# Repeerc/flash-attention-v2-RDNA3-minimal

Hardware: AMD Instinct MI355X
Metric: fwd attention TFLOPS (and % MFMA roofline) at B2 H16 N4096 D128 fp16 (higher is better)
Workload: dtype f16; 1 GPU; c2: B2 H16 N4096 D128 float16 causal=False per GPU, BHND, torch.rand U[0,1); global_batch=2, parallelism=batch-shard x1 (no data-path collective)

## Files before the change

### flash-attention-v2-rdna3-minimal_amd/build.py

```python
import argparse
import concurrent.futures
import fcntl
import hashlib
import os
import shutil
import subprocess
import sys
import tempfile

PKG_DIR = os.path.dirname(os.path.realpath(__file__))
REPO_ROOT = os.path.dirname(PKG_DIR)
CSRC = os.path.join(PKG_DIR, "csrc")
INCLUDE = os.path.join(REPO_ROOT, "include")
LIB_NAME = "libfa2_gfx950.so"
LIB_PATH = os.path.join(PKG_DIR, LIB_NAME)
STAMP_PATH = LIB_PATH + ".stamp"
LOCK_PATH = LIB_PATH + ".lock"

UNITS = [
    ("host", "host.cpp", []),
    ("fwd_hip_f16", "fwd_hip.cpp", ["-DFA2_TU_BF16=0"]),
    ("fwd_hip_bf16", "fwd_hip.cpp", ["-DFA2_TU_BF16=1"]),
    ("fwd_hip_trim_f16", "fwd_hip.cpp", ["-DFA2_TU_BF16=0", "-DFA2_TU_TRIM=1"]),
    ("fwd_hip_trim_bf16", "fwd_hip.cpp", ["-DFA2_TU_BF16=1", "-DFA2_TU_TRIM=1"]),
    ("fwd_asm", "fwd_asm.cpp", []),
    ("bwd_hip_f16", "bwd_hip.cpp", ["-DFA2_TU_BF16=0"]),
    ("bwd_hip_bf16", "bwd_hip.cpp", ["-DFA2_TU_BF16=1"]),
    ("bwd_hip_trim_f16", "bwd_hip.cpp", ["-DFA2_TU_BF16=0", "-DFA2_TU_TRIM=1"]),
    ("bwd_hip_trim_bf16", "bwd_hip.cpp", ["-DFA2_TU_BF16=1", "-DFA2_TU_TRIM=1"]),
    ("bwd_asm", "bwd_asm.cpp", []),
    ("bwd_bias_hip_f16", "bwd_bias_hip.cpp", ["-DFA2_TU_BF16=0"]),
    ("bwd_bias_hip_bf16", "bwd_bias_hip.cpp", ["-DFA2_TU_BF16=1"]),
    ("window_hip_f16", "window_hip.cpp", ["-DFA2_TU_BF16=0"]),
    ("window_hip_bf16", "window_hip.cpp", ["-DFA2_TU_BF16=1"]),
    ("varlen_hip_f16", "varlen_hip.cpp", ["-DFA2_TU_BF16=0"]),
    ("varlen_hip_bf16", "varlen_hip.cpp", ["-DFA2_TU_BF16=1"]),
    ("dropout_hip_f16", "dropout_hip.cpp", ["-DFA2_TU_BF16=0"]),
    ("dropout_hip_bf16", "dropout_hip.cpp", ["-DFA2_TU_BF16=1"]),
    ("varlen_dropout_hip_f16", "varlen_dropout_hip.cpp", ["-DFA2_TU_BF16=0"]),
    ("varlen_dropout_hip_bf16", "varlen_dropout_hip.cpp", ["-DFA2_TU_BF16=1"]),
    ("scoremod_hip_f16", "scoremod_hip.cpp", ["-DFA2_TU_BF16=0"]),
    ("scoremod_hip_bf16", "scoremod_hip.cpp", ["-DFA2_TU_BF16=1"]),
    ("varlen_scoremod_hip_f16", "varlen_scoremod_hip.cpp", ["-DFA2_TU_BF16=0"]),
    ("varlen_scoremod_hip_bf16", "varlen_scoremod_hip.cpp", ["-DFA2_TU_BF16=1"]),
]
FRONTEND_SRC = "frontend.cpp"
FRONTEND_PATH = os.path.join(PKG_DIR, "rocwmma_fattn", "_fa2_frontend.so")
GENERATORS = [os.path.join("gen", "fwd_d128_gen.py"), os.path.join("gen", "fwd_m16_gen.py"), os.path.join("gen", "fwd_m16_d256_gen.py"), os.path.join("gen", "bwd_d128_gen.py"),
              os.path.join("gen", "bwd_dq_m16_gen.py"), os.path.join("gen", "bwd_dkv_m16_gen.py")]
HEADERS = ["fa2_launch.h", "fa2_window.h", "fa2_dropout.h", "fa2_scoremod.h", "fa2_fwd_kernel.hip.h", "fa2_fwd_short.hip.h", "fa2_fwd_d128.hip.h", "fa2_fwd_d256.hip.h", "fa2_bwd_kernel.hip.h", "fa2_bwd_short.hip.h", "fa2_bwd_d128.hip.h",
           os.path.join(INCLUDE, "fa2_gfx950.h"), os.path.join("gen", "isa.py"), os.path.join("gen", "sched.py")] + GENERATORS

HIPCC_FLAGS = [
    "-x", "hip",
    "--offload-arch=gfx950",
    "-O3",
    "-std=c++17",
    "-fPIC",
    "-fvisibility-inlines-hidden",
    "-fno-honor-nans",
    "--offload-compress",
]


def _hipcc():
    for cand in (os.environ.get("HIPCC"), shutil.which("hipcc"), "/opt/rocm/bin/hipcc"):
        if cand and os.path.exists(cand):
            return cand
    raise RuntimeError("hipcc not found (set HIPCC or install ROCm); the gfx950 library cannot be built")


def _existing(names):
    out = []
    for name in names:
        path = name if os.path.isabs(name) else os.path.join(CSRC, name)
        if os.path.exists(path):
            out.append(path)
    return out


def _source_digest():
    h = hashlib.sha256()
    h.update(" ".join(HIPCC_FLAGS).encode())
    for (obj, src, flags) in UNITS:
        h.update(("%s %s %s" % (obj, src, " ".join(flags))).encode())
    for path in _existing(sorted(set(u[1] for u in UNITS)) + HEADERS + [FRONTEND_SRC]):
        with open(path, "rb") as f:
            h.update(f.read())
    return h.hexdigest()


def _dir_digest(d):
    h = hashlib.sha256()
    for name in sorted(os.listdir(d)):
        if name.endswith(".inc"):
            h.update(name.encode())
            with open(os.path.join(d, name), "rb") as f:
                h.update(f.read())
    return h.hexdigest()


def generate(out_dir=None, opts=None, probe=False):
    out_dir = out_dir or CSRC
# ... 136 lines not shown
```

### flash-attention-v2-rdna3-minimal_amd/csrc/fa2_fwd_d128.hip.h

```cpp
#pragma once
#include "fa2_fwd_kernel.hip.h"

#ifndef FA2_D128_INC_DIR
#define FA2_D128_INC(name) #name
#else
#define FA2_D128_STR2(x) #x
#define FA2_D128_STR(x) FA2_D128_STR2(x)
#define FA2_D128_INC(name) FA2_D128_STR(FA2_D128_INC_DIR/name)
#endif

namespace fa2 {

template <int HD>
struct AsmGeo {
    static constexpr int ROWB = 2 * HD, TILEB = 64 * ROWB;
    static constexpr int EPI_ROWB = ROWB + 16;
    static constexpr int EPI_BASE = 4 * TILEB;
    static constexpr int FAIL_OFF = EPI_BASE + 4 * 64 * EPI_ROWB;
    static constexpr int LDS_BYTES = FAIL_OFF + 16;
    static constexpr int RPP = 1024 / ROWB;
};
constexpr int kD128LdsBytes = AsmGeo<128>::LDS_BYTES;

typedef uint32_t u32x4s __attribute__((ext_vector_type(4)));

struct D128Item {
    u32x4s qrs, krs, vrs;
    uint32_t qw;
    int lim[2];
    int ntw, ntiles;
    int b, h, qw0;
    int slot;
};

__device__ __forceinline__ int part_of_item(const FwdParams& p, int v, int& item, int& part) {
    item = v;
    part = -1;
    if (p.nsplit > 1 && v >= p.full_items) {
        const int j = v - p.full_items;
        part = j / p.split_items;
        item = p.full_items + j % p.split_items;
        return (j % p.split_items) * p.nsplit + part;
    }
    return -1;
}


__device__ __forceinline__ void causal_item(const FwdParams& p, int v, int& bh, int& qblk) {
    const int P = (p.nqblk + 1) >> 1;
    const int unit = v >> 1, part = v & 1;
    int head, i;
    if ((p.nbh & 7) == 0) { const int r = unit >> 3; head = (unit & 7) + 8 * (r / P); i = r % P; }
    else { head = unit / P; i = unit % P; }
    bh = head + p.bh0;
    qblk = part ? i : p.nqblk - 1 - i;
}
__device__ __forceinline__ bool causal_unit_has_second(const FwdParams& p, int v) {
    const int P = (p.nqblk + 1) >> 1, unit = v >> 1;
    const int i = ((p.nbh & 7) == 0 ? unit >> 3 : unit) % P;
    return 2 * i + 1 < p.nqblk;
}
template <int HD, bool BF16, bool CAUSAL, bool FOLD, bool M16 = false, bool LM = false>
__global__ __launch_bounds__(256, 1) void fwd_asm_kernel(const FwdParams p_in) {
    using AG = AsmGeo<HD>;
    using G_ = Geo<HD, 4>;
    extern __shared__ __attribute__((aligned(16))) char smem[];
    int vb = blockIdx.x;
    if constexpr (CAUSAL) {
        if (p_in.persist != 0) vb = 2 * blockIdx.x;
    }
#ifdef FA2_STAMP
    const uint64_t stamp0 = __builtin_amdgcn_s_memrealtime();
    const uint64_t cyc0 = __builtin_readcyclecounter();
#endif
    uint32_t staged = 0;
    if (threadIdx.x < 4) reinterpret_cast<volatile uint32_t*>(smem + AG::FAIL_OFF)[threadIdx.x] = 0;
    __syncthreads();
#pragma clang loop unroll(disable)
    do {
        int tid = threadIdx.x;
        asm volatile("" : "+v"(tid), "+s"(staged));
        const FwdParams& p = p_in;
        const int lane = tid & 63;
        const int wave = __builtin_amdgcn_readfirstlane(tid >> 6);
        const int l31 = lane & 31, hi = lane >> 5;
        int nitems = (CAUSAL && p.persist != 0) ? 2 * p.nbh * ((p.nqblk + 1) >> 1) : p.nbh * p.nqblk;
        if (!CAUSAL && p.item_cap > 0) nitems = p.item_cap;

        const uint32_t k_rowb = (uint32_t)p.ks[2] * 2u, v_rowb = (uint32_t)p.vs[2] * 2u, q_rowb = (uint32_t)p.qs[2] * 2u;
        const int drow = 16 * wave + lane / G_::G, dslot = lane % G_::G;
        const uint32_t kd0 = drow * k_rowb + ((dslot ^ ((drow / G_::RPB) & G_::KMASK)) << 4);
        const int qrow = lane / G_::G;
        const uint32_t qd0 = qrow * q_rowb + ((dslot ^ ((qrow / G_::RPB) & G_::KMASK)) << 4);
        const uint32_t q_t16 = 16u * q_rowb;
        const uint32_t vd0 = drow * v_rowb + (((((dslot >> 2) ^ ((drow / G_::RPB) & G_::VMASK)) << 2) |
                                               ((dslot & 3) ^ ((M16 && (FOLD || LM)) ? (((drow >> 2) & 1) << 1) : 0))) << 4);
        const int pp4 = lane & 15, g1 = (lane >> 4) & 1;
        const int n16 = lane & 15, g4 = lane >> 4;
        const int trow16 = 4 * g4 + (n16 >> 2);
        const uint32_t kr0 = M16 ? (uint32_t)(n16 * AG::ROWB + ((g4 ^ ((n16 / G_::RPB) & G_::KMASK)) << 4)) : (uint32_t)G_::k_off(l31, hi);
        const uint32_t vr0 = M16 ? (uint32_t)(trow16 * AG::ROWB + (((trow16 / G_::RPB) & G_::VMASK) << 6) + 8 * (n16 & 3) + ((FOLD || LM) ? 32 * (g4 & 1) : 0))
                                 : (uint32_t)G_::v_off(4 * hi + (pp4 >> 2), 32 * g1 + 8 * (pp4 & 3));
        const uint32_t epi = M16 ? AG::EPI_BASE + wave * 64 * AG::EPI_ROWB + n16 * AG::EPI_ROWB + g4 * 8
                                 : AG::EPI_BASE + wave * 64 * AG::EPI_ROWB + l31 * AG::EPI_ROWB + hi * 16;
        const uint32_t k_tile = kKvTile * k_rowb, v_tile = kKvTile * v_rowb, k_row4 = AG::RPP * k_rowb - 1024, v_row4 = AG::RPP * v_rowb - 1024;
        const uint32_t ldsw = wave * (AG::TILEB / 4);
        const float c = p.c;

        auto make_item = [&](int item) {
            D128Item it;
            int bh, qblk;
            int kv_first = 0, nkv = p.Nkv;
            it.slot = -1;
            if constexpr (CAUSAL) {
                if (p.persist != 0) causal_item(p, item, bh, qblk);
                else block_to_head_qblock<CAUSAL>(p, item, bh, qblk);
            } else {
                int whole, part;
                it.slot = part_of_item(p, item, whole, part);
                block_to_head_qblock<CAUSAL>(p, whole, bh, qblk);
                if (part >= 0) {
                    const int nt = (p.Nkv + kKvTile - 1) / kKvTile;
                    const int t0 = part * nt / p.nsplit, t1 = (part + 1) * nt / p.nsplit;
                    kv_first = t0 * kKvTile;
                    nkv = (t1 * kKvTile < p.Nkv ? t1 * kKvTile : p.Nkv) - kv_first;
                }
                kv_first = __builtin_amdgcn_readfirstlane(kv_first);
                nkv = __builtin_amdgcn_readfirstlane(nkv);
                bh = __builtin_amdgcn_readfirstlane(bh);
                qblk = __builtin_amdgcn_readfirstlane(qblk);
                it.slot = __builtin_amdgcn_readfirstlane(it.slot);
            }
            it.b = bh / p.H;
            it.h = bh % p.H;
            const int q0 = qblk * 256;
            it.qw0 = q0 + wave * 64;
            int ntiles = (nkv + kKvTile - 1) / kKvTile;
            if (CAUSAL) {
                const int qmax = (q0 + 256 < p.Nq ? q0 + 256 : p.Nq) - 1;
                const int nt_c = qmax / kKvTile + 1;
                ntiles = nt_c < ntiles ? nt_c : ntiles;
            }
            int ntw = ntiles;
            if (CAUSAL) {
                const int nt_w = (it.qw0 + 63) / kKvTile + 1;
                ntw = nt_w < ntiles ? nt_w : ntiles;
            }
            it.ntiles = ntiles;
            it.ntw = ntw;
            const uint64_t qa = (uint64_t)((const uint16_t*)p.q + it.b * p.qs[0] + it.h * p.qs[1]);
            it.qrs = (u32x4s){(uint32_t)qa, (uint32_t)(qa >> 32) & 0xffffu, (uint32_t)(p.Nq - 1) * q_rowb + 2u * (uint32_t)p.D, 0x00020000u};
            it.qw = __builtin_amdgcn_readfirstlane(it.qw0 < p.Nq ? (uint32_t)it.qw0 * q_rowb : 0u);
#pragma unroll
            for (int qb = 0; qb < 2; ++qb) {
                const int qrow = it.qw0 + 32 * qb + l31;
                const int lim_c = CAUSAL ? qrow : 0x3fffffff;
                it.lim[qb] = (lim_c < nkv - 1 ? lim_c : nkv - 1) - kKvTile * (ntw - 1) - 4 * hi;
            }
            if constexpr (M16) {
                it.lim[0] = (CAUSAL ? it.qw0 + n16 : 0x3fff0000) - kKvTile * (ntw - 1) - 4 * g4;
                it.lim[1] = nkv - 1 - kKvTile * (ntw - 1) - 4 * g4;
            }
            const uint64_t ka = (uint64_t)((const uint16_t*)p.k + it.b * p.ks[0] + (it.h / p.kv_group) * p.ks[1] + (int64_t)kv_first * p.ks[2]);
            const uint64_t va = (uint64_t)((const uint16_t*)p.v + it.b * p.vs[0] + (it.h / p.kv_group) * p.vs[1] + (int64_t)kv_first * p.vs[2]);
            it.krs = (u32x4s){(uint32_t)ka, (uint32_t)(ka >> 32) & 0xffffu, p.k_bytes - (uint32_t)kv_first * k_rowb, 0x00020000u};
            it.vrs = (u32x4s){(uint32_t)va, (uint32_t)(va >> 32) & 0xffffu, p.v_bytes - (uint32_t)kv_first * v_rowb, 0x00020000u};
            return it;
        };

        int nvb;
        if constexpr (CAUSAL) {
            if (p.persist == 0) nvb = nitems;
            else if (!(vb & 1) && causal_unit_has_second(p, vb)) nvb = vb + 1;
            else nvb = (vb | 1) - 1 + 2 * (int)gridDim.x;
        } else {
            nvb = vb + (int)gridDim.x;
        }
        const bool has_next = nvb < nitems;
        const D128Item cur = make_item(vb);
        const D128Item nxt = make_item(has_next ? nvb : vb);
        const uint32_t flags = __builtin_amdgcn_readfirstlane(staged | (has_next ? 2u : 0u) | (nxt.ntiles >= 2 ? 4u : 0u) | (cur.slot >= 0 ? 8u : 0u) |
                                                              ((M16 && p.D < HD) ? (uint32_t)(p.D >> 3) << 8 : 0u));
        const int slot_u = __builtin_amdgcn_readfirstlane(cur.slot >= 0 ? cur.slot : 0);
        const uint64_t ws_tile = (uint64_t)(p.ws + (int64_t)slot_u * kSplitRows * HD);
        float lse0, lse1;

#define FA2_D128_OPERANDS                                                                                              \
    : "=v"(lse0), "=v"(lse1)                                                                                           \
    : "v"(qd0), "s"(cur.qw), "s"(cur.qrs), "s"(cur.krs), "s"(cur.vrs), "v"(kd0), "v"(vd0), "v"(kr0), "v"(vr0), \
      "v"(cur.lim[0]), "v"(cur.lim[1]), "s"(c), "s"(cur.ntw), "s"(cur.ntiles), "s"(k_tile), "s"(v_tile), "s"(k_row4),    \
      "s"(v_row4), "s"(ldsw), "v"(epi), "s"(flags), "s"(nxt.qw), "s"(q_t16), "s"(nxt.qrs), "s"(nxt.krs),                \
      "s"(nxt.vrs), "s"(ws_tile)                                                                                        \
    :
        if constexpr (M16 && LM && !FOLD) {
            if constexpr (HD == 64 && BF16) {
                asm volatile(
#include FA2_D128_INC(fa2_fwd_m16_d64_bf16_lm.inc)
                    FA2_D128_OPERANDS
#include FA2_D128_INC(fa2_fwd_d128_clobbers.inc)
                );
            } else if constexpr (HD == 64) {
                asm volatile(
#include FA2_D128_INC(fa2_fwd_m16_d64_f16_lm.inc)
                    FA2_D128_OPERANDS
#include FA2_D128_INC(fa2_fwd_d128_clobbers.inc)
                );
            } else if constexpr (BF16) {
                asm volatile(
#include FA2_D128_INC(fa2_fwd_m16_bf16_lm.inc)
                    FA2_D128_OPERANDS
#include FA2_D128_INC(fa2_fwd_d128_clobbers.inc)
                );
            } else {
                asm volatile(
#include FA2_D128_INC(fa2_fwd_m16_f16_lm.inc)
                    FA2_D128_OPERANDS
#include FA2_D128_INC(fa2_fwd_d128_clobbers.inc)
                );
            }
        } else if constexpr (M16 && HD == 64 && BF16 && FOLD) {
            asm volatile(
#include FA2_D128_INC(fa2_fwd_m16_d64_bf16_fold.inc)
                FA2_D128_OPERANDS
#include FA2_D128_INC(fa2_fwd_d128_clobbers.inc)
            );
        } else if constexpr (M16 && HD == 64 && FOLD) {
            asm volatile(
#include FA2_D128_INC(fa2_fwd_m16_d64_f16_fold.inc)
                FA2_D128_OPERANDS
#include FA2_D128_INC(fa2_fwd_d128_clobbers.inc)
            );
        } else if constexpr (M16 && HD == 64 && BF16) {
            asm volatile(
#include FA2_D128_INC(fa2_fwd_m16_d64_bf16.inc)
                FA2_D128_OPERANDS
#include FA2_D128_INC(fa2_fwd_d128_clobbers.inc)
            );
        } else if constexpr (M16 && HD == 64) {
            asm volatile(
#include FA2_D128_INC(fa2_fwd_m16_d64_f16.inc)
                FA2_D128_OPERANDS
#include FA2_D128_INC(fa2_fwd_d128_clobbers.inc)
            );
// ... 33 lines not shown
                FA2_D128_OPERANDS
#include FA2_D128_INC(fa2_fwd_d128_clobbers.inc)
            );
        } else if constexpr (HD == 128 && BF16 && FOLD) {
            asm volatile(
#include FA2_D128_INC(fa2_fwd_d128_bf16_fold.inc)
                FA2_D128_OPERANDS
#include FA2_D128_INC(fa2_fwd_d128_clobbers.inc)
            );
        } else if constexpr (HD == 128 && BF16) {
            asm volatile(
#include FA2_D128_INC(fa2_fwd_d128_bf16.inc)
                FA2_D128_OPERANDS
#include FA2_D128_INC(fa2_fwd_d128_clobbers.inc)
            );
        } else if constexpr (HD == 128 && FOLD) {
            asm volatile(
#include FA2_D128_INC(fa2_fwd_d128_f16_fold.inc)
                FA2_D128_OPERANDS
#include FA2_D128_INC(fa2_fwd_d128_clobbers.inc)
            );
        } else if constexpr (HD == 128) {
            asm volatile(
#include FA2_D128_INC(fa2_fwd_d128_f16.inc)
                FA2_D128_OPERANDS
#include FA2_D128_INC(fa2_fwd_d128_clobbers.inc)
            );
        } else if constexpr (BF16 && FOLD) {
            asm volatile(
#include FA2_D128_INC(fa2_fwd_d64_bf16_fold.inc)
                FA2_D128_OPERANDS
#include FA2_D128_INC(fa2_fwd_d128_clobbers.inc)
            );
        } else if constexpr (BF16) {
            asm volatile(
#include FA2_D128_INC(fa2_fwd_d64_bf16.inc)
                FA2_D128_OPERANDS
#include FA2_D128_INC(fa2_fwd_d128_clobbers.inc)
            );
        } else if constexpr (FOLD) {
            asm volatile(
#include FA2_D128_INC(fa2_fwd_d64_f16_fold.inc)
                FA2_D128_OPERANDS
#include FA2_D128_INC(fa2_fwd_d128_clobbers.inc)
            );
        } else {
            asm volatile(
#include FA2_D128_INC(fa2_fwd_d64_f16.inc)
                FA2_D128_OPERANDS
#include FA2_D128_INC(fa2_fwd_d128_clobbers.inc)
            );
        }
#undef FA2_D128_OPERANDS

        int tid2 = threadIdx.x, item2 = vb;
        asm volatile("" : "+v"(tid2));
        {
            if constexpr (M16) __syncthreads();
            const u32x4 fw = *reinterpret_cast<const volatile u32x4*>(smem + AG::FAIL_OFF);
            const uint32_t fany = __builtin_amdgcn_readfirstlane(fw.x | fw.y | fw.z | fw.w);
            if (fany != 0) {
                __syncthreads();
                if (tid2 < 4) reinterpret_cast<volatile uint32_t*>(smem + AG::FAIL_OFF)[tid2] = 0;
                __syncthreads();
            }
            if ((fany & 1u) == 0 && fany != 0) staged = __builtin_amdgcn_readfirstlane(staged | 32u);
            if ((fany & 1u) != 0) {
                staged = __builtin_amdgcn_readfirstlane(16u | 32u);
                continue;
            }
        }
        {
            const FwdParams& p2 = p_in;
            const int lane2 = tid2 & 63, wave2 = __builtin_amdgcn_readfirstlane(tid2 >> 6);
            int bh, qblk, slot2 = -1;
            if constexpr (CAUSAL) {
                if (p2.persist != 0) causal_item(p2, item2, bh, qblk);
                else block_to_head_qblock<CAUSAL>(p2, item2, bh, qblk);
            } else {
                int whole, part;
                slot2 = part_of_item(p2, item2, whole, part);
                block_to_head_qblock<CAUSAL>(p2, whole, bh, qblk);
            }
            const int b = bh / p2.H, h = bh % p2.H;
            const int qw0 = qblk * 256 + wave2 * 64;
            {
                const bool is_part = slot2 >= 0;
                float* lp = is_part ? p2.ws + (int64_t)p2.split_items * p2.nsplit * kSplitRows * HD + (int64_t)slot2 * kSplitRows + wave2 * 64 - qw0
                                    : p2.lse + b * p2.ls[0] + h * p2.ls[1];
                if constexpr (M16) {
                    if (is_part || qw0 + lane2 < p2.Nq) lp[qw0 + lane2] = lse0;
                } else if ((lane2 >> 5) == 0) {
                    if (is_part || qw0 + (lane2 & 31) < p2.Nq) lp[qw0 + (lane2 & 31)] = lse0;
                    if (is_part || qw0 + 32 + (lane2 & 31) < p2.Nq) lp[qw0 + 32 + (lane2 & 31)] = lse1;
                }
            }
            const int nq_store = slot2 >= 0 ? 0 : p2.Nq;
            const char* img = smem + AG::EPI_BASE + wave2 * 64 * AG::EPI_ROWB;
            constexpr int LPR = HD / 8;
            const int rl = lane2 / LPR, cl = lane2 % LPR;
            uint16_t* obase = (uint16_t*)p2.o + b * p2.os[0] + h * p2.os[1];
#pragma unroll
            for (int i = 0; i < 64 / (64 / LPR); ++i) {
                const int r = i * (64 / LPR) + rl;
                const u32x4 w = *(const u32x4*)(img + r * AG::EPI_ROWB + cl * 16);
#ifdef FA2_O_NT
                if (qw0 + r < nq_store) __builtin_nontemporal_store(w, (u32x4*)(obase + (int64_t)(qw0 + r) * p2.os[2] + cl * 8));
#else
                if (qw0 + r < nq_store && cl * 8 < p2.D) *(u32x4*)(obase + (int64_t)(qw0 + r) * p2.os[2] + cl * 8) = w;
#endif
            }
            staged = __builtin_amdgcn_readfirstlane((has_next ? 1u : 0u) | ((staged & 32u) ? 48u : 0u));
            vb = nvb;
#ifdef FA2_STAMP
            if (!has_next && lane2 == 0) {
                __builtin_amdgcn_s_waitcnt(0);
                uint64_t* st = (uint64_t*)p2.lse + (blockIdx.x * 4 + wave2) * 4;
                st[0] = stamp0;
                st[1] = __builtin_amdgcn_s_memrealtime();
                st[2] = __builtin_readcyclecounter() - cyc0;
                st[3] = ((uint64_t)__builtin_amdgcn_s_getreg(6164) << 32) | __builtin_amdgcn_s_getreg(63492);
            }
#endif
            if (!has_next) break;
        }
    } while (true);
}

}
```

### flash-attention-v2-rdna3-minimal_amd/csrc/fa2_fwd_kernel.hip.h

```cpp
#pragma once
#include <hip/hip_runtime.h>
#include <stdint.h>
#include <type_traits>

#include "fa2_window.h"

#ifndef FA2_WIN
#define FA2_WIN 0
#endif
#ifndef FA2_VARLEN
#define FA2_VARLEN 0
#endif
#if FA2_VARLEN && !FA2_WIN
#error "FA2_VARLEN builds on the FA2_WIN blocks"
#endif
#if FA2_VARLEN
#define FA2_KP pk
#else
#define FA2_KP p
#endif
#ifndef FA2_DROP
#define FA2_DROP 0
#endif
#if FA2_DROP && !FA2_WIN
#error "FA2_DROP builds on the FA2_WIN blocks"
#endif
#if FA2_DROP
#include "fa2_dropout.h"
#endif
#ifndef FA2_SMOD
#define FA2_SMOD 0
#endif
#if FA2_SMOD && (!FA2_WIN || FA2_DROP)
#error "FA2_SMOD builds on the FA2_WIN blocks and does not combine with FA2_DROP"
#endif
#if FA2_SMOD
#include "fa2_scoremod.h"
#define FA2_SMOD_PARAM , const ScoreMod smod
#else
#define FA2_SMOD_PARAM
#endif

#ifndef FA2_DEFER_THR
#define FA2_DEFER_THR 8.0f
#endif
#ifndef FA2_LDS_DMA
#define FA2_LDS_DMA 1
#endif
#ifndef FA2_LDS_DMA_MIN_HD
#define FA2_LDS_DMA_MIN_HD 128
#endif
#ifndef FA2_EPI_LDS
#define FA2_EPI_LDS 1
#endif
#ifndef FA2_IGLP
#define FA2_IGLP 0
#endif
#ifndef FA2_TILE_IN_SOFFSET
#define FA2_TILE_IN_SOFFSET 1
#endif
#if FA2_TILE_IN_SOFFSET
#define FA2_TILE_OFF(voff, soff) (voff), (soff)
#else
#define FA2_TILE_OFF(voff, soff) (voff) + (soff), 0u
#endif

namespace fa2 {

typedef _Float16 f16x8 __attribute__((ext_vector_type(8)));
typedef __bf16 bf16x8 __attribute__((ext_vector_type(8)));
typedef _Float16 f16x2 __attribute__((ext_vector_type(2)));
typedef __bf16 bf16x2 __attribute__((ext_vector_type(2)));
typedef float f32x16 __attribute__((ext_vector_type(16)));
typedef float f32x2 __attribute__((ext_vector_type(2)));
typedef float f32x4 __attribute__((ext_vector_type(4)));
typedef uint32_t u32x4 __attribute__((ext_vector_type(4)));
typedef uint32_t u32x2 __attribute__((ext_vector_type(2)));
typedef short s16x4 __attribute__((ext_vector_type(4)));
typedef uint32_t u32x32 __attribute__((ext_vector_type(32)));

constexpr int kQBlock = 256;
constexpr int kKvTile = 64;
constexpr uint32_t kOobOffset = 0x80000000u;

struct FwdParams {
    const void* q;
    const void* k;
    const void* v;
    void* o;
    float* lse;
    int B, H, Nq, Nkv;
    int D;
    int64_t qs[3], ks[3], vs[3], os[3];
    int64_t ls[2];
    float c;
    int negate_q;
    int nqblk;
    uint32_t k_bytes, v_bytes;
    int bh0, nbh;
    int rows_hint;
    int exact_scale;
    int persist;
    const void* bias;
    int64_t bs[3];
    int bias_kind;
    int bias_vec;
    int full_items, split_items, nsplit;
    int blk0;
    int item_cap;
    float* ws;
    int kv_group = 1;
};

template <typename P>
__host__ __device__ inline void set_window(P& p, const Window& w) { p.bs[0] = w.left; p.bs[1] = w.right; p.bs[2] = w.off; }
template <typename P>
__host__ __device__ inline Window get_window(const P& p) {
    Window w;
    w.left = (int)p.bs[0]; w.right = (int)p.bs[1]; w.off = (int)p.bs[2];
    return w;
}
struct VarlenPtrs { const int* cu_q; const int* cu_k; };
template <typename P>
__host__ __device__ inline void set_varlen(P& p, const int* cu_q, const int* cu_k) { p.bias = cu_q; p.ws = (float*)const_cast<int*>(cu_k); }
template <typename P>
__host__ __device__ inline VarlenPtrs get_varlen(const P& p) { return {(const int*)p.bias, (const int*)p.ws}; }

#if FA2_VARLEN
struct VarlenSeq { int q_base, k_base, Nq, Nkv; };
template <typename P>
__device__ __forceinline__ VarlenSeq varlen_seq(const P& p, int s) {
    const int *cq = get_varlen(p).cu_q, *ck = get_varlen(p).cu_k;
    VarlenSeq v;
    v.q_base = cq[s]; v.k_base = ck[s];
    v.Nq = cq[s + 1] - v.q_base; v.Nkv = ck[s + 1] - v.k_base;
    return v;
}
__device__ __forceinline__ uint32_t varlen_bytes(int n, int64_t pitch, int D) { return n > 0 ? (uint32_t)(((int64_t)(n - 1) * pitch + D) * 2) : 0u; }
__device__ __forceinline__ bool varlen_enter(FwdParams& p, Window& win, int s, int row0) {
    const VarlenSeq v = varlen_seq(p, s);
    if (row0 >= v.Nq) return true;
    p.Nq = v.Nq; p.Nkv = v.Nkv;
    win.off = win.off ? v.Nkv - v.Nq : 0;
    p.q = (const uint16_t*)p.q + (int64_t)v.q_base * p.qs[2];
    p.k = (const uint16_t*)p.k + (int64_t)v.k_base * p.ks[2];
    p.v = (const uint16_t*)p.v + (int64_t)v.k_base * p.vs[2];
    p.o = (uint16_t*)p.o + (int64_t)v.q_base * p.os[2];
    p.lse += v.q_base;
    p.k_bytes = varlen_bytes(v.Nkv, p.ks[2], p.D);
    p.v_bytes = varlen_bytes(v.Nkv, p.vs[2], p.D);
    return false;
}
#endif

constexpr int kSplitRows = 256;
constexpr int kMaxSplit = 8;

__host__ __device__ inline int64_t split_ws_bytes(int split_items, int nsplit, int HD) {
    return (int64_t)split_items * nsplit * kSplitRows * (HD + 1) * 4;
}

template <bool BF16>
__device__ __forceinline__ f32x16 mfma16(u32x4 a, u32x4 b, f32x16 c) {
    if constexpr (BF16)
// ... 958 lines not shown
```

### flash-attention-v2-rdna3-minimal_amd/csrc/fwd_asm.cpp

```cpp
#include "fa2_launch.h"

#include "fa2_fwd_d128.hip.h"
#include "fa2_fwd_d256.hip.h"
#include "fa2_gfx950.h"

namespace {

template <int HD, bool BF16, bool CAUSAL, bool FOLD, bool M16 = false, bool LM = false>
int launch_asm_t(const fa2::FwdParams& p0, hipStream_t stream) {
    constexpr auto kern = fa2::fwd_asm_kernel<HD, BF16, CAUSAL, FOLD, M16, LM>;
    constexpr int lds = fa2::AsmGeo<HD>::LDS_BYTES;
    if (int rc = fa2::set_lds<kern>(lds)) return rc;
    fa2::FwdParams p = p0;
    p.persist = fa2::options().persist.load(std::memory_order_relaxed) ? 1 : 0;
    const int pg = fa2::device_cus() & ~7;
    if (CAUSAL && p.persist) {
        const int64_t units = (int64_t)p.nbh * ((p.nqblk + 1) / 2);
#if defined(FA2_PAIRS_ROUND4)
        if (!(units > pg || p.nqblk >= 32)) p.persist = 0;
#elif !defined(FA2_PAIRS_ALWAYS)
        if (!(units >= pg || p.nqblk >= 32)) p.persist = 0;
#endif
    }
    const int64_t per_head = (CAUSAL && p.persist) ? (p.nqblk + 1) / 2 : p.nqblk;
    int64_t grid = (int64_t)p.nbh * per_head;
    if (!CAUSAL && p.item_cap > 0) grid = p.item_cap;
    if (p.persist && pg > 0 && grid > pg) grid = pg;
    hipLaunchKernelGGL(kern, dim3((unsigned)grid), dim3(256), lds, stream, p);
    return (int)hipGetLastError();
}

template <bool BF16, bool CAUSAL, bool TRIM, int KS = 8>
int launch_d256_t(const fa2::FwdParams& p0, hipStream_t stream) {
    constexpr auto kern = fa2::fwd_asm_d256_kernel<BF16, CAUSAL, TRIM, KS>;
    if (int rc = fa2::set_lds<kern>(fa2::kD256LdsBytes)) return rc;
    fa2::FwdParams p = p0;
    p.nqblk = (p.Nq + fa2::kD256Rows - 1) / fa2::kD256Rows;
    const int64_t grid = (int64_t)p.nbh * p.nqblk;
    if (grid > 0x7fffffffLL) return FA2_ERR_GRID;
    hipLaunchKernelGGL(kern, dim3((unsigned)grid), dim3(256), fa2::kD256LdsBytes, stream, p);
    return (int)hipGetLastError();
}

}

namespace fa2 {

int launch_fwd_asm_d256(bool bf16, const FwdParams& p, bool causal, hipStream_t stream) {
    if (p.D < 256) {
        const int ks = (p.D + 31) / 32;
#define FA2_D256_TRIM_CASE(K)                                                                                                              \
        if (ks == K) {                                                                                                                 \
            if (bf16) return causal ? launch_d256_t<true, true, true, K>(p, stream) : launch_d256_t<true, false, true, K>(p, stream);   \
            return causal ? launch_d256_t<false, true, true, K>(p, stream) : launch_d256_t<false, false, true, K>(p, stream);           \
        }
        FA2_D256_TRIM_CASE(5) FA2_D256_TRIM_CASE(6) FA2_D256_TRIM_CASE(7) FA2_D256_TRIM_CASE(8)
#undef FA2_D256_TRIM_CASE
        return FA2_ERR_HEAD_DIM;
    }
    if (bf16) return causal ? launch_d256_t<true, true, false>(p, stream) : launch_d256_t<true, false, false>(p, stream);
    return causal ? launch_d256_t<false, true, false>(p, stream) : launch_d256_t<false, false, false>(p, stream);
}

template <int HD, bool BF16>
static int launch_asm_hd(const FwdParams& p, bool causal, bool fold, hipStream_t stream) {
    if (fold) return causal ? launch_asm_t<HD, BF16, true, true>(p, stream) : launch_asm_t<HD, BF16, false, true>(p, stream);
    return causal ? launch_asm_t<HD, BF16, true, false>(p, stream) : launch_asm_t<HD, BF16, false, false>(p, stream);
}

int launch_fwd_asm(int HD, bool bf16, const FwdParams& p, bool causal, bool fold, hipStream_t stream, int m16) {
    const int kind = fwd_asm_m16_kind(HD, bf16, p, fold, m16);
    if (kind == kM16F32Lm) {
        if (HD == 64) {
            if (bf16) return causal ? launch_asm_t<64, true, true, false, true, true>(p, stream) : launch_asm_t<64, true, false, false, true, true>(p, stream);
            return causal ? launch_asm_t<64, false, true, false, true, true>(p, stream) : launch_asm_t<64, false, false, false, true, true>(p, stream);
        }
        if (bf16) return causal ? launch_asm_t<128, true, true, false, true, true>(p, stream) : launch_asm_t<128, true, false, false, true, true>(p, stream);
        return causal ? launch_asm_t<128, false, true, false, true, true>(p, stream) : launch_asm_t<128, false, false, false, true, true>(p, stream);
    }
    if (HD == 64 && kind != kM16None) {
// ... 21 lines not shown
```

Baseline: 1427 TFLOPS.

## Step persistent work-item positions incrementally and carry next item across loop iterations

Adds a shared item-map header that decodes an item index into batch/head/kv-head/qblock once, then advances it by a precomputed host-side stride delta instead of redoing divisions and modulos per iteration. The persistent loop now builds the next item only once and reuses it as the current one, rather than recomputing both every trip. The epilogue reuses cached output and LSE row pointers and batches the output stores three at a time. The aim is to cut scalar index arithmetic and epilogue latency between tiles, at the cost of more loop-carried state and register pressure.

```diff
diff --git a/flash-attention-v2-rdna3-minimal_amd/build.py b/flash-attention-v2-rdna3-minimal_amd/build.py
--- a/flash-attention-v2-rdna3-minimal_amd/build.py
+++ b/flash-attention-v2-rdna3-minimal_amd/build.py
@@ -48,7 +48,7 @@
 FRONTEND_PATH = os.path.join(PKG_DIR, "rocwmma_fattn", "_fa2_frontend.so")
 GENERATORS = [os.path.join("gen", "fwd_d128_gen.py"), os.path.join("gen", "fwd_m16_gen.py"), os.path.join("gen", "fwd_m16_d256_gen.py"), os.path.join("gen", "bwd_d128_gen.py"),
               os.path.join("gen", "bwd_dq_m16_gen.py"), os.path.join("gen", "bwd_dkv_m16_gen.py")]
-HEADERS = ["fa2_launch.h", "fa2_window.h", "fa2_dropout.h", "fa2_scoremod.h", "fa2_fwd_kernel.hip.h", "fa2_fwd_short.hip.h", "fa2_fwd_d128.hip.h", "fa2_fwd_d256.hip.h", "fa2_bwd_kernel.hip.h", "fa2_bwd_short.hip.h", "fa2_bwd_d128.hip.h",
+HEADERS = ["fa2_launch.h", "fa2_window.h", "fa2_dropout.h", "fa2_scoremod.h", "fa2_item_map.h", "fa2_fwd_kernel.hip.h", "fa2_fwd_short.hip.h", "fa2_fwd_d128.hip.h", "fa2_fwd_d256.hip.h", "fa2_bwd_kernel.hip.h", "fa2_bwd_short.hip.h", "fa2_bwd_d128.hip.h",
            os.path.join(INCLUDE, "fa2_gfx950.h"), os.path.join("gen", "isa.py"), os.path.join("gen", "sched.py")] + GENERATORS
 
 HIPCC_FLAGS = [
diff --git a/flash-attention-v2-rdna3-minimal_amd/csrc/fa2_fwd_d128.hip.h b/flash-attention-v2-rdna3-minimal_amd/csrc/fa2_fwd_d128.hip.h
--- a/flash-attention-v2-rdna3-minimal_amd/csrc/fa2_fwd_d128.hip.h
+++ b/flash-attention-v2-rdna3-minimal_amd/csrc/fa2_fwd_d128.hip.h
@@ -1,5 +1,6 @@
 #pragma once
 #include "fa2_fwd_kernel.hip.h"
+#include "fa2_item_map.h"
 
 #ifndef FA2_D128_INC_DIR
 #define FA2_D128_INC(name) #name
@@ -27,51 +28,76 @@
 struct D128Item {
     u32x4s qrs, krs, vrs;
     uint32_t qw;
-    int lim[2];
     int ntw, ntiles;
-    int b, h, qw0;
+    int nkv;
+    int qw0;
     int slot;
+    uint16_t* orow;
+    float* lrow;
 };
 
-__device__ __forceinline__ int part_of_item(const FwdParams& p, int v, int& item, int& part) {
-    item = v;
-    part = -1;
-    if (p.nsplit > 1 && v >= p.full_items) {
-        const int j = v - p.full_items;
-        part = j / p.split_items;
-        item = p.full_items + j % p.split_items;
-        return (j % p.split_items) * p.nsplit + part;
-    }
-    return -1;
-}
-
-
-__device__ __forceinline__ void causal_item(const FwdParams& p, int v, int& bh, int& qblk) {
-    const int P = (p.nqblk + 1) >> 1;
-    const int unit = v >> 1, part = v & 1;
-    int head, i;
-    if ((p.nbh & 7) == 0) { const int r = unit >> 3; head = (unit & 7) + 8 * (r / P); i = r % P; }
-    else { head = unit / P; i = unit % P; }
-    bh = head + p.bh0;
-    qblk = part ? i : p.nqblk - 1 - i;
-}
-__device__ __forceinline__ bool causal_unit_has_second(const FwdParams& p, int v) {
-    const int P = (p.nqblk + 1) >> 1, unit = v >> 1;
-    const int i = ((p.nbh & 7) == 0 ? unit >> 3 : unit) % P;
-    return 2 * i + 1 < p.nqblk;
-}
+
 template <int HD, bool BF16, bool CAUSAL, bool FOLD, bool M16 = false, bool LM = false>
 __global__ __launch_bounds__(256, 1) void fwd_asm_kernel(const FwdParams p_in) {
     using AG = AsmGeo<HD>;
     using G_ = Geo<HD, 4>;
     extern __shared__ __attribute__((aligned(16))) char smem[];
-    int vb = blockIdx.x;
-    if constexpr (CAUSAL) {
-        if (p_in.persist != 0) vb = 2 * blockIdx.x;
-    }
+    const FwdParams& p = p_in;
+    const int stride = (int)gridDim.x;
+    const int nitems = item_count(p, CAUSAL);
+    auto uniform = [](ItemPos q) {
+        q.v = __builtin_amdgcn_readfirstlane(q.v); q.pih = __builtin_amdgcn_readfirstlane(q.pih); q.b = __builtin_amdgcn_readfirstlane(q.b);
+        q.h = __builtin_amdgcn_readfirstlane(q.h); q.hkv = __builtin_amdgcn_readfirstlane(q.hkv); q.hr = __builtin_amdgcn_readfirstlane(q.hr);
+        q.qblk = __builtin_amdgcn_readfirstlane(q.qblk); q.part = __builtin_amdgcn_readfirstlane(q.part); q.slot = __builtin_amdgcn_readfirstlane(q.slot);
+        return q;
+    };
+    ItemPos pos = uniform(item_closed<CAUSAL>(p, (CAUSAL && p.persist != 0) ? 2 * (int)blockIdx.x : (int)blockIdx.x));
+    const int wave = __builtin_amdgcn_readfirstlane((int)threadIdx.x >> 6);
+    auto make_item = [&](const ItemPos& at) {
+        D128Item it;
+        const uint32_t k_rowb = (uint32_t)p.ks[2] * 2u, v_rowb = (uint32_t)p.vs[2] * 2u, q_rowb = (uint32_t)p.qs[2] * 2u;
+        int kv_first = 0, nkv = p.Nkv;
+        it.slot = at.slot;
+        if (!CAUSAL && at.part >= 0) {
+            const int nt = (p.Nkv + kKvTile - 1) / kKvTile;
+            const int t0 = at.part * nt / p.nsplit, t1 = (at.part + 1) * nt / p.nsplit;
+            kv_first = __builtin_amdgcn_readfirstlane(t0 * kKvTile);
+            nkv = __builtin_amdgcn_readfirstlane((t1 * kKvTile < p.Nkv ? t1 * kKvTile : p.Nkv) - kv_first);
+        }
+        const int q0 = at.qblk * 256;
+        it.qw0 = q0 + wave * 64;
+        int ntiles = (nkv + kKvTile - 1) / kKvTile;
+        if (CAUSAL) {
+            const int qmax = (q0 + 256 < p.Nq ? q0 + 256 : p.Nq) - 1;
+            const int nt_c = qmax / kKvTile + 1;
+            ntiles = nt_c < ntiles ? nt_c : ntiles;
+        }
+        int ntw = ntiles;
+        if (CAUSAL) {
+            const int nt_w = (it.qw0 + 63) / kKvTile + 1;
+            ntw = nt_w < ntiles ? nt_w : ntiles;
+        }
+        it.ntiles = ntiles;
+        it.ntw = ntw;
+        it.nkv = nkv;
+        const uint64_t qa = (uint64_t)((const uint16_t*)p.q + at.b * p.qs[0] + at.h * p.qs[1]);
+        it.qrs = (u32x4s){(uint32_t)qa, (uint32_t)(qa >> 32) & 0xffffu, (uint32_t)(p.Nq - 1) * q_rowb + 2u * (uint32_t)p.D, 0x00020000u};
+        it.qw = it.qw0 < p.Nq ? (uint32_t)it.qw0 * q_rowb : 0u;
+        const uint64_t ka = (uint64_t)((const uint16_t*)p.k + at.b * p.ks[0] + at.hkv * p.ks[1] + (int64_t)kv_first * p.ks[2]);
+        const uint64_t va = (uint64_t)((const uint16_t*)p.v + at.b * p.vs[0] + at.hkv * p.vs[1] + (int64_t)kv_first * p.vs[2]);
+        it.krs = (u32x4s){(uint32_t)ka, (uint32_t)(ka >> 32) & 0xffffu, p.k_bytes - (uint32_t)kv_first * k_rowb, 0x00020000u};
+        it.vrs = (u32x4s){(uint32_t)va, (uint32_t)(va >> 32) & 0xffffu, p.v_bytes - (uint32_t)kv_first * v_rowb, 0x00020000u};
+        it.orow = (uint16_t*)p.o + at.b * p.os[0] + at.h * p.os[1] + (int64_t)it.qw0 * p.os[2];
+        it.lrow = at.slot >= 0 ? p.ws + (int64_t)p.split_items * p.nsplit * kSplitRows * HD + (int64_t)at.slot * kSplitRows + wave * 64 - it.qw0
+                               : p.lse + at.b * p.ls[0] + at.h * p.ls[1];
+        return it;
+    };
+    D128Item cur = make_item(pos);
 #ifdef FA2_STAMP
     const uint64_t stamp0 = __builtin_amdgcn_s_memrealtime();
     const uint64_t cyc0 = __builtin_readcyclecounter();
+    uint64_t cyc_mark = cyc0, cyc_shell = 0, cyc_stmt = 0;
+    uint32_t trips = 0;
 #endif
     uint32_t staged = 0;
     if (threadIdx.x < 4) reinterpret_cast<volatile uint32_t*>(smem + AG::FAIL_OFF)[threadIdx.x] = 0;
@@ -80,12 +106,8 @@
     do {
         int tid = threadIdx.x;
         asm volatile("" : "+v"(tid), "+s"(staged));
-        const FwdParams& p = p_in;
         const int lane = tid & 63;
-        const int wave = __builtin_amdgcn_readfirstlane(tid >> 6);
         const int l31 = lane & 31, hi = lane >> 5;
-        int nitems = (CAUSAL && p.persist != 0) ? 2 * p.nbh * ((p.nqblk + 1) >> 1) : p.nbh * p.nqblk;
-        if (!CAUSAL && p.item_cap > 0) nitems = p.item_cap;
 
         const uint32_t k_rowb = (uint32_t)p.ks[2] * 2u, v_rowb = (uint32_t)p.vs[2] * 2u, q_rowb = (uint32_t)p.qs[2] * 2u;
         const int drow = 16 * wave + lane / G_::G, dslot = lane % G_::G;
@@ -107,88 +129,38 @@
         const uint32_t ldsw = wave * (AG::TILEB / 4);
         const float c = p.c;
 
-        auto make_item = [&](int item) {
-            D128Item it;
-            int bh, qblk;
-            int kv_first = 0, nkv = p.Nkv;
-            it.slot = -1;
-            if constexpr (CAUSAL) {
-                if (p.persist != 0) causal_item(p, item, bh, qblk);
-                else block_to_head_qblock<CAUSAL>(p, item, bh, qblk);
-            } else {
-                int whole, part;
-                it.slot = part_of_item(p, item, whole, part);
-                block_to_head_qblock<CAUSAL>(p, whole, bh, qblk);
-                if (part >= 0) {
-                    const int nt = (p.Nkv + kKvTile - 1) / kKvTile;
-                    const int t0 = part * nt / p.nsplit, t1 = (part + 1) * nt / p.nsplit;
-                    kv_first = t0 * kKvTile;
-                    nkv = (t1 * kKvTile < p.Nkv ? t1 * kKvTile : p.Nkv) - kv_first;
-                }
-                kv_first = __builtin_amdgcn_readfirstlane(kv_first);
-                nkv = __builtin_amdgcn_readfirstlane(nkv);
-                bh = __builtin_amdgcn_readfirstlane(bh);
-                qblk = __builtin_amdgcn_readfirstlane(qblk);
-                it.slot = __builtin_amdgcn_readfirstlane(it.slot);
-            }
-            it.b = bh / p.H;
-            it.h = bh % p.H;
-            const int q0 = qblk * 256;
-            it.qw0 = q0 + wave * 64;
-            int ntiles = (nkv + kKvTile - 1) / kKvTile;
-            if (CAUSAL) {
-                const int qmax = (q0 + 256 < p.Nq ? q0 + 256 : p.Nq) - 1;
-                const int nt_c = qmax / kKvTile + 1;
-                ntiles = nt_c < ntiles ? nt_c : ntiles;
-            }
-            int ntw = ntiles;
-            if (CAUSAL) {
-                const int nt_w = (it.qw0 + 63) / kKvTile + 1;
-                ntw = nt_w < ntiles ? nt_w : ntiles;
-            }
-            it.ntiles = ntiles;
-            it.ntw = ntw;
-            const uint64_t qa = (uint64_t)((const uint16_t*)p.q + it.b * p.qs[0] + it.h * p.qs[1]);
-            it.qrs = (u32x4s){(uint32_t)qa, (uint32_t)(qa >> 32) & 0xffffu, (uint32_t)(p.Nq - 1) * q_rowb + 2u * (uint32_t)p.D, 0x00020000u};
-            it.qw = __builtin_amdgcn_readfirstlane(it.qw0 < p.Nq ? (uint32_t)it.qw0 * q_rowb : 0u);
+        ItemPos npos = pos;
+        const int stepped = item_try_step<CAUSAL>(p, p.steps, nitems, stride, npos);
+        if (stepped == 2) npos = uniform(item_closed<CAUSAL>(p, npos.v));
+        const bool has_next = stepped != 0;
+        D128Item nxt = cur;
+        if (has_next) nxt = make_item(npos);
+        int lim[2];
 #pragma unroll
-            for (int qb = 0; qb < 2; ++qb) {
-                const int qrow = it.qw0 + 32 * qb + l31;
-                const int lim_c = CAUSAL ? qrow : 0x3fffffff;
-                it.lim[qb] = (lim_c < nkv - 1 ? lim_c : nkv - 1) - kKvTile * (ntw - 1) - 4 * hi;
-            }
-            if constexpr (M16) {
-                it.lim[0] = (CAUSAL ? it.qw0 + n16 : 0x3fff0000) - kKvTile * (ntw - 1) - 4 * g4;
-                it.lim[1] = nkv - 1 - kKvTile * (ntw - 1) - 4 * g4;
-            }
-            const uint64_t ka = (uint64_t)((const uint16_t*)p.k + it.b * p.ks[0] + (it.h / p.kv_group) * p.ks[1] + (int64_t)kv_first * p.ks[2]);
-            const uint64_t va = (uint64_t)((const uint16_t*)p.v + it.b * p.vs[0] + (it.h / p.kv_group) * p.vs[1] + (int64_t)kv_first * p.vs[2]);
-            it.krs = (u32x4s){(uint32_t)ka, (uint32_t)(ka >> 32) & 0xffffu, p.k_bytes - (uint32_t)kv_first * k_rowb, 0x00020000u};
-            it.vrs = (u32x4s){(uint32_t)va, (uint32_t)(va >> 32) & 0xffffu, p.v_bytes - (uint32_t)kv_first * v_rowb, 0x00020000u};
-            return it;
-        };
-
-        int nvb;
-        if constexpr (CAUSAL) {
-            if (p.persist == 0) nvb = nitems;
-            else if (!(vb & 1) && causal_unit_has_second(p, vb)) nvb = vb + 1;
-            else nvb = (vb | 1) - 1 + 2 * (int)gridDim.x;
-        } else {
-            nvb = vb + (int)gridDim.x;
-        }
-        const bool has_next = nvb < nitems;
-        const D128Item cur = make_item(vb);
-        const D128Item nxt = make_item(has_next ? nvb : vb);
+        for (int qb = 0; qb < 2; ++qb) {
+            const int lim_c = CAUSAL ? cur.qw0 + 32 * qb + l31 : 0x3fffffff;
+            lim[qb] = (lim_c < cur.nkv - 1 ? lim_c : cur.nkv - 1) - kKvTile * (cur.ntw - 1) - 4 * hi;
+        }
+        if constexpr (M16) {
+            lim[0] = (CAUSAL ? cur.qw0 + n16 : 0x3fff0000) - kKvTile * (cur.ntw - 1) - 4 * g4;
+            lim[1] = cur.nkv - 1 - kKvTile * (cur.ntw - 1) - 4 * g4;
+        }
         const uint32_t flags = __builtin_amdgcn_readfirstlane(staged | (has_next ? 2u : 0u) | (nxt.ntiles >= 2 ? 4u : 0u) | (cur.slot >= 0 ? 8u : 0u) |
                                                               ((M16 && p.D < HD) ? (uint32_t)(p.D >> 3) << 8 : 0u));
-        const int slot_u = __builtin_amdgcn_readfirstlane(cur.slot >= 0 ? cur.slot : 0);
-        const uint64_t ws_tile = (uint64_t)(p.ws + (int64_t)slot_u * kSplitRows * HD);
+        const uint64_t ws_tile = (uint64_t)(p.ws + (int64_t)(cur.slot >= 0 ? cur.slot : 0) * kSplitRows * HD);
         float lse0, lse1;
+#ifdef FA2_STAMP
+        {
+            const uint64_t t = __builtin_readcyclecounter();
+            cyc_shell += t - cyc_mark;
+            cyc_mark = t;
+        }
+#endif
 
 #define FA2_D128_OPERANDS                                                                                              \
     : "=v"(lse0), "=v"(lse1)                                                                                           \
     : "v"(qd0), "s"(cur.qw), "s"(cur.qrs), "s"(cur.krs), "s"(cur.vrs), "v"(kd0), "v"(vd0), "v"(kr0), "v"(vr0), \
-      "v"(cur.lim[0]), "v"(cur.lim[1]), "s"(c), "s"(cur.ntw), "s"(cur.ntiles), "s"(k_tile), "s"(v_tile), "s"(k_row4),    \
+      "v"(lim[0]), "v"(lim[1]), "s"(c), "s"(cur.ntw), "s"(cur.ntiles), "s"(k_tile), "s"(v_tile), "s"(k_row4),    \
       "s"(v_row4), "s"(ldsw), "v"(epi), "s"(flags), "s"(nxt.qw), "s"(q_t16), "s"(nxt.qrs), "s"(nxt.krs),                \
       "s"(nxt.vrs), "s"(ws_tile)                                                                                        \
     :
@@ -328,8 +300,16 @@
             );
         }
 #undef FA2_D128_OPERANDS
-
-        int tid2 = threadIdx.x, item2 = vb;
+#ifdef FA2_STAMP
+        {
+            const uint64_t t = __builtin_readcyclecounter();
+            cyc_stmt += t - cyc_mark;
+            cyc_mark = t;
+            ++trips;
+        }
+#endif
+
+        int tid2 = threadIdx.x;
         asm volatile("" : "+v"(tid2));
         {
             if constexpr (M16) __syncthreads();
@@ -347,58 +327,73 @@
             }
         }
         {
-            const FwdParams& p2 = p_in;
-            const int lane2 = tid2 & 63, wave2 = __builtin_amdgcn_readfirstlane(tid2 >> 6);
-            int bh, qblk, slot2 = -1;
-            if constexpr (CAUSAL) {
-                if (p2.persist != 0) causal_item(p2, item2, bh, qblk);
-                else block_to_head_qblock<CAUSAL>(p2, item2, bh, qblk);
-            } else {
-                int whole, part;
-                slot2 = part_of_item(p2, item2, whole, part);
-                block_to_head_qblock<CAUSAL>(p2, whole, bh, qblk);
-            }
-            const int b = bh / p2.H, h = bh % p2.H;
-            const int qw0 = qblk * 256 + wave2 * 64;
+            const int lane2 = tid2 & 63;
+            const bool is_part = cur.slot >= 0;
+            const int qw0 = cur.qw0;
             {
-                const bool is_part = slot2 >= 0;
-                float* lp = is_part ? p2.ws + (int64_t)p2.split_items * p2.nsplit * kSplitRows * HD + (int64_t)slot2 * kSplitRows + wave2 * 64 - qw0
-                                    : p2.lse + b * p2.ls[0] + h * p2.ls[1];
+                float* lp = cur.lrow;
                 if constexpr (M16) {
-                    if (is_part || qw0 + lane2 < p2.Nq) lp[qw0 + lane2] = lse0;
+                    if (is_part || qw0 + lane2 < p.Nq) lp[qw0 + lane2] = lse0;
                 } else if ((lane2 >> 5) == 0) {
-                    if (is_part || qw0 + (lane2 & 31) < p2.Nq) lp[qw0 + (lane2 & 31)] = lse0;
-                    if (is_part || qw0 + 32 + (lane2 & 31) < p2.Nq) lp[qw0 + 32 + (lane2 & 31)] = lse1;
+                    if (is_part || qw0 + (lane2 & 31) < p.Nq) lp[qw0 + (lane2 & 31)] = lse0;
+                    if (is_part || qw0 + 32 + (lane2 & 31) < p.Nq) lp[qw0 + 32 + (lane2 & 31)] = lse1;
                 }
             }
-            const int nq_store = slot2 >= 0 ? 0 : p2.Nq;
-            const char* img = smem + AG::EPI_BASE + wave2 * 64 * AG::EPI_ROWB;
+            const int nq_store = is_part ? 0 : p.Nq;
+            const char* img = smem + AG::EPI_BASE + wave * 64 * AG::EPI_ROWB;
             constexpr int LPR = HD / 8;
+            constexpr int RPI = 64 / LPR, NI = 64 / RPI;
             const int rl = lane2 / LPR, cl = lane2 % LPR;
-            uint16_t* obase = (uint16_t*)p2.o + b * p2.os[0] + h * p2.os[1];
+            const char* src = img + rl * AG::EPI_ROWB + cl * 16;
+#ifndef FA2_O_NT
+            if (!is_part && qw0 + 64 <= p.Nq && p.D == HD && (uint64_t)p.os[2] < (1u << 24)) {
+                char* ob = (char*)cur.orow;
+                const uint32_t loff = (uint32_t)rl * ((uint32_t)p.os[2] * 2u) + (uint32_t)cl * 16u;
+                const int64_t pitch = (int64_t)RPI * p.os[2] * 2;
 #pragma unroll
-            for (int i = 0; i < 64 / (64 / LPR); ++i) {
-                const int r = i * (64 / LPR) + rl;
-                const u32x4 w = *(const u32x4*)(img + r * AG::EPI_ROWB + cl * 16);
+                for (int i0 = 0; i0 < NI; i0 += 3) {
+                    u32x4 w[3];
+#pragma unroll
+                    for (int j = 0; j < 3; ++j)
+                        if (i0 + j < NI) w[j] = *(const u32x4*)(src + (i0 + j) * RPI * AG::EPI_ROWB);
+#pragma unroll
+                    for (int j = 0; j < 3; ++j)
+                        if (i0 + j < NI) *(u32x4*)(ob + (i0 + j) * pitch + loff) = w[j];
+                }
+            } else
+#endif
+            {
+                uint16_t* obase = cur.orow + (int64_t)rl * p.os[2] + cl * 8;
+#pragma unroll
+                for (int i = 0; i < NI; ++i) {
+                    const int r = i * RPI + rl;
+                    const u32x4 w = *(const u32x4*)(src + i * RPI * AG::EPI_ROWB);
 #ifdef FA2_O_NT
-                if (qw0 + r < nq_store) __builtin_nontemporal_store(w, (u32x4*)(obase + (int64_t)(qw0 + r) * p2.os[2] + cl * 8));
+                    if (qw0 + r < nq_store) __builtin_nontemporal_store(w, (u32x4*)(obase + (int64_t)(i * RPI) * p.os[2]));
 #else
-                if (qw0 + r < nq_store && cl * 8 < p2.D) *(u32x4*)(obase + (int64_t)(qw0 + r) * p2.os[2] + cl * 8) = w;
-#endif
+                    if (qw0 + r < nq_store && cl * 8 < p.D) *(u32x4*)(obase + (int64_t)(i * RPI) * p.os[2]) = w;
+#endif
+                }
             }
             staged = __builtin_amdgcn_readfirstlane((has_next ? 1u : 0u) | ((staged & 32u) ? 48u : 0u));
-            vb = nvb;
 #ifdef FA2_STAMP
             if (!has_next && lane2 == 0) {
                 __builtin_amdgcn_s_waitcnt(0);
-                uint64_t* st = (uint64_t*)p2.lse + (blockIdx.x * 4 + wave2) * 4;
+                uint64_t* st = (uint64_t*)p.lse + (blockIdx.x * 4 + wave) * 8;
+                const uint64_t cyc1 = __builtin_readcyclecounter();
                 st[0] = stamp0;
                 st[1] = __builtin_amdgcn_s_memrealtime();
-                st[2] = __builtin_readcyclecounter() - cyc0;
+                st[2] = cyc1 - cyc0;
                 st[3] = ((uint64_t)__builtin_amdgcn_s_getreg(6164) << 32) | __builtin_amdgcn_s_getreg(63492);
+                st[4] = cyc_shell + (cyc1 - cyc_mark);
+                st[5] = cyc_stmt;
+                st[6] = trips;
+                st[7] = 0;
             }
 #endif
             if (!has_next) break;
+            cur = nxt;
+            pos = npos;
         }
     } while (true);
 }
diff --git a/flash-attention-v2-rdna3-minimal_amd/csrc/fa2_fwd_kernel.hip.h b/flash-attention-v2-rdna3-minimal_amd/csrc/fa2_fwd_kernel.hip.h
--- a/flash-attention-v2-rdna3-minimal_amd/csrc/fa2_fwd_kernel.hip.h
+++ b/flash-attention-v2-rdna3-minimal_amd/csrc/fa2_fwd_kernel.hip.h
@@ -4,6 +4,7 @@
 #include <type_traits>
 
 #include "fa2_window.h"
+#include "fa2_item_map.h"
 
 #ifndef FA2_WIN
 #define FA2_WIN 0
@@ -110,6 +111,7 @@
     int item_cap;
     float* ws;
     int kv_group = 1;
+    ItemSteps steps = {};
 };
 
 template <typename P>
diff --git a/flash-attention-v2-rdna3-minimal_amd/csrc/fa2_item_map.h b/flash-attention-v2-rdna3-minimal_amd/csrc/fa2_item_map.h
--- /dev/null
+++ b/flash-attention-v2-rdna3-minimal_amd/csrc/fa2_item_map.h
@@ -0,0 +1,150 @@
+#pragma once
+
+#if defined(__HIPCC__) || defined(__CUDACC__)
+#define FA2_MAP_FN __host__ __device__ inline
+#else
+#define FA2_MAP_FN inline
+#endif
+
+#ifndef FA2_CAUSAL_HPG
+#define FA2_CAUSAL_HPG 0
+#endif
+
+namespace fa2 {
+
+struct HeadStep { int db, dh, dkv, dr; };
+
+struct ItemSteps {
+    int q_step;
+    int per_head;
+    int hkv_n;
+    HeadStep whole;
+    HeadStep carry;
+};
+
+struct ItemPos {
+    int v;
+    int pih;
+    int b, h, hkv, hr;
+    int qblk;
+    int part, slot;
+};
+
+template <class P>
+FA2_MAP_FN int item_count(const P& p, bool causal) {
+    if (causal) return p.persist != 0 ? 2 * p.nbh * ((p.nqblk + 1) >> 1) : p.nbh * p.nqblk;
+    return p.item_cap > 0 ? p.item_cap : p.nbh * p.nqblk;
+}
+
+FA2_MAP_FN HeadStep make_head_step(int d, int H, int kv_group) {
+    HeadStep s;
+    s.db = d / H;
+    s.dh = d % H;
+    s.dkv = s.dh / kv_group;
+    s.dr = s.dh % kv_group;
+    return s;
+}
+
+template <class P>
+FA2_MAP_FN ItemSteps make_item_steps(const P& p, bool causal, int stride) {
+    ItemSteps s;
+    const bool x8 = (p.nbh & 7) == 0;
+    s.per_head = (causal && p.persist != 0) ? (p.nqblk + 1) >> 1 : p.nqblk;
+    s.hkv_n = p.H / p.kv_group;
+    const int rows = x8 ? stride >> 3 : stride, hm = x8 ? 8 : 1;
+    s.q_step = (x8 && (stride & 7) != 0) ? -1 : rows % s.per_head;
+    s.whole = make_head_step(hm * (rows / s.per_head), p.H, p.kv_group);
+    s.carry = make_head_step(hm, p.H, p.kv_group);
+    return s;
+}
+
+template <class P>
+FA2_MAP_FN void item_set_head(const P& p, int bh, ItemPos& pos) {
+    pos.b = bh / p.H;
+    pos.h = bh % p.H;
+    pos.hkv = pos.h / p.kv_group;
+    pos.hr = pos.h % p.kv_group;
+}
+
+template <bool CAUSAL, class P>
+FA2_MAP_FN ItemPos item_closed(const P& p, int v) {
+    ItemPos pos;
+    pos.v = v;
+    pos.part = pos.slot = -1;
+    const bool x8 = (p.nbh & 7) == 0;
+    int head;
+    if (CAUSAL && p.persist == 0) {
+        if (x8) {
+            const int slot = v >> 3, hpx = p.nbh >> 3;
+            constexpr int kHpg = FA2_CAUSAL_HPG > 0 ? FA2_CAUSAL_HPG : 1;
+            const int hpg = (FA2_CAUSAL_HPG > 0 && hpx % kHpg == 0) ? kHpg : hpx;
+            const int per_group = hpg * p.nqblk, g = slot / per_group, r = slot % per_group;
+            head = (v & 7) + 8 * (g * hpg + r % hpg);
+            pos.pih = r / hpg;
+        } else {
+            head = v % p.nbh;
+            pos.pih = v / p.nbh;
+        }
+        pos.qblk = p.nqblk - 1 - pos.pih;
+    } else {
+        int u = CAUSAL ? v >> 1 : v;
+        const int per_head = CAUSAL ? (p.nqblk + 1) >> 1 : p.nqblk;
+        if (!CAUSAL && p.nsplit > 1 && v >= p.full_items) {
+            const int j = v - p.full_items;
+            pos.part = j / p.split_items;
+            u = p.full_items + j % p.split_items;
+            pos.slot = (j % p.split_items) * p.nsplit + pos.part;
+        }
+        if (x8) { head = (u & 7) + 8 * ((u >> 3) / per_head); pos.pih = (u >> 3) % per_head; }
+        else { head = u / per_head; pos.pih = u % per_head; }
+        pos.qblk = !CAUSAL ? pos.pih : (v & 1) ? pos.pih : p.nqblk - 1 - pos.pih;
+    }
+    item_set_head(p, head + p.bh0, pos);
+    return pos;
+}
+
+template <class P>
+FA2_MAP_FN void item_add_heads(const P& p, const ItemSteps& s, const HeadStep& d, ItemPos& pos) {
+    pos.b += d.db;
+    pos.h += d.dh;
+    pos.hkv += d.dkv;
+    pos.hr += d.dr;
+    if (pos.hr >= p.kv_group) { pos.hr -= p.kv_group; ++pos.hkv; }
+    if (pos.h >= p.H) { pos.h -= p.H; pos.hkv -= s.hkv_n; ++pos.b; }
+}
+
+template <bool CAUSAL, class P>
+FA2_MAP_FN int item_try_step(const P& p, const ItemSteps& s, int nitems, int stride, ItemPos& pos) {
+    int nv;
+    if (CAUSAL) {
+        if (p.persist == 0) return 0;
+        if (!(pos.v & 1) && 2 * pos.pih + 1 < p.nqblk) {
+            ++pos.v;
+            pos.qblk = pos.pih;
+            return 1;
+        }
+        nv = (pos.v | 1) - 1 + 2 * stride;
+    } else {
+        nv = pos.v + stride;
+    }
+    if (nv >= nitems) return 0;
+    pos.v = nv;
+    if (s.q_step < 0 || (!CAUSAL && p.nsplit > 1 && nv >= p.full_items)) return 2;
+    pos.pih += s.q_step;
+    item_add_heads(p, s, s.whole, pos);
+    if (pos.pih >= s.per_head) {
+        pos.pih -= s.per_head;
+        item_add_heads(p, s, s.carry, pos);
+    }
+    pos.qblk = CAUSAL ? p.nqblk - 1 - pos.pih : pos.pih;
+    return 1;
+}
+
+template <bool CAUSAL, class P>
+FA2_MAP_FN bool item_step(const P& p, const ItemSteps& s, int nitems, int stride, ItemPos& pos) {
+    const int r = item_try_step<CAUSAL>(p, s, nitems, stride, pos);
+    if (r == 2) pos = item_closed<CAUSAL>(p, pos.v);
+    return r != 0;
+}
+
+}
diff --git a/flash-attention-v2-rdna3-minimal_amd/csrc/fwd_asm.cpp b/flash-attention-v2-rdna3-minimal_amd/csrc/fwd_asm.cpp
--- a/flash-attention-v2-rdna3-minimal_amd/csrc/fwd_asm.cpp
+++ b/flash-attention-v2-rdna3-minimal_amd/csrc/fwd_asm.cpp
@@ -26,6 +26,7 @@
     int64_t grid = (int64_t)p.nbh * per_head;
     if (!CAUSAL && p.item_cap > 0) grid = p.item_cap;
     if (p.persist && pg > 0 && grid > pg) grid = pg;
+    p.steps = fa2::make_item_steps(p, CAUSAL, (int)grid);
     hipLaunchKernelGGL(kern, dim3((unsigned)grid), dim3(256), lds, stream, p);
     return (int)hipGetLastError();
 }
```

Result: no change. 1427 TFLOPS (-0.0%).
